# weihaoysgs/ssvio

Measured on AMD Instinct MI355X. Metric: stereo frames/s (ORB extract + row-band match + triangulate + one local BA per frame) on 1241x376, higher is better.
Workload: dtype u8 (front-end) + f64 (BA)

## Files before the change

ssvio_amd/csrc/ba.hip:

```cpp
#include <algorithm>
#include <atomic>
#include <chrono>
#include <cmath>
#include <limits>
#include <map>
#include <condition_variable>
#include <functional>
#include <mutex>
#include <numeric>
#include <thread>
#include <unordered_map>
#include <vector>

#include <cstring>
#include <rocprim/device/device_radix_sort.hpp>
#include <rocprim/device/device_run_length_encode.hpp>
#include <rocprim/device/device_scan.hpp>

#include "ctx.hpp"
#include "se3.hpp"
#include "../../include/ssx_test_hooks.h"

int ssx_comm_allreduce_f64(void* user, double* buf_dev, size_t count, void* stream);

// ... 45 lines not shown
using gcdouble_p = const double*;
#endif


struct BaDev {
  int P, L, E, nP, nLm, nCh, nBlk, world, rank;
  int big;
  int store_w;
  int lin_stride;
  int dense_slabs;
  GPtr<unsigned int> touch;
  GPtr<const int> pose_free;
  GPtr<const uint8_t> lm_fixed;
  GPtr<const int> lm_id;
  GPtr<const int> lm_ptr;
  GPtr<const int> ch_lm;
  GPtr<const int> e_pose;
  GPtr<const int> e_lmc;
  GPtr<const uint8_t> e_cam;
  GPtr<const uint8_t> e_dup;
  GPtr<const double> e_uv;
  GPtr<const int8_t> blk_pa;
  GPtr<const int8_t> blk_pb;
  GPtr<const int4> ch_desc;
  GPtr<const int4> e_rec;
  GPtr<const int4> l_rec;
  GPtr<const uint16_t> pptr;
  GPtr<uint8_t> pair_a;
  GPtr<uint8_t> pair_b;
  GPtr<int> pair_ptr;
  GPtr<int4> bseg;
  GPtr<int> bseg_ptr;
  int bseg_cap;
  int dev_prep;
  int E_raw;
  GPtr<const int> r_edge_pose;
  GPtr<const int> r_edge_point;
  GPtr<const double> r_edge_uv;
  GPtr<const uint8_t> r_edge_cam;
  GPtr<const uint8_t> r_slot8;
  int no_err;
  int raw_fmt;
  GPtr<const int> lm_compact;
  GPtr<const int> pose_rank;
  GPtr<int> perm;
  GPtr<int> lm_chunk;
// ... 134 lines not shown

template <int K0, int N>
__device__ __forceinline__ void pose_terms(const double* Ji, double w, double r0, double r1, double* V)
{
  int k = 0;
#pragma unroll
  for (int r = 0; r < 6; ++r)
#pragma unroll
    for (int cc = r; cc < 6; ++cc) {
      if (k >= K0 && k < K0 + N) V[k - K0] = Ji[r] * w * Ji[cc] + Ji[6 + r] * w * Ji[6 + cc];
      ++k;
    }
#pragma unroll
  for (int a = 0; a < 6; ++a) {
    if (k >= K0 && k < K0 + N) V[k - K0] = Ji[a] * r0 + Ji[6 + a] * r1;
    ++k;
  }
}

__device__ __forceinline__ double run_sum(const double* row, int s0, int s1)
{
  double acc = 0.0;
  int s = s0;
  for (; s < s1; s += 8) {
    double v[8];
#pragma unroll
    for (int i = 0; i < 8; ++i) v[i] = row[s + i];
#pragma unroll
    for (int i = 0; i < 8; ++i) acc += (s + i < s1) ? v[i] : 0.0;
  }
  return acc;
}

__device__ __forceinline__ bool chunk_touches(const BaDev& d, int c, int bit)
{
  return d.dense_slabs || ((d.touch[(size_t)c * TOUCH_WORDS + (bit >> 5)] >> (bit & 31)) & 1u);
}

template <int JAC>
__device__ __forceinline__ void k_linearize_body(const BaDev& d, const int bx, int cur, char* smem, const ChunkLists& cl, double* Wout, double* lmout,
                                                 int* erw_out, double* slab)
{
  double (*sL)[CH_E + 1] = reinterpret_cast<double (*)[CH_E + 1]>(smem);
  double* sV = reinterpret_cast<double*>(smem) + 9 * (CH_E + 1);
  double* sRed = reinterpret_cast<double*>(smem);
  const uint16_t* sPptr = reinterpret_cast<const uint16_t*>(smem + BA_OFF_PPTR);

// ... 603 lines not shown
  if (!both) {
#pragma unroll
    for (int k = 0; k < 18; ++k) W[k] = 0.0;
    return;
  }
  const double* pose = d.pose[cur];
  const double* point = d.point[cur];
  double T[7], X[3];
#pragma unroll
  for (int k = 0; k < 7; ++k) T[k] = pose[p * 7 + k];
#pragma unroll
  for (int k = 0; k < 3; ++k) X[k] = point[lid * 3 + k];
  const double* ext = d.ext + 7 * (er4.w & 1);
  double er[2], p1[3], pc[3], Ji[12], Jj[6], rho0, w;
  ssx::edge_error(T, X, ext, d.K, d.e_uv[e], d.e_uv[d.E + e], er, p1, pc);
  ssx::edge_jac_analytic(T, ext, d.K, p1, pc, Ji, Jj);
  ssx::huber(er[0] * er[0] + er[1] * er[1], d.huber_delta, rho0, w);
#pragma unroll
  for (int a = 0; a < 6; ++a)
#pragma unroll
    for (int b = 0; b < 3; ++b) W[a * 3 + b] = Ji[a] * w * Jj[b] + Ji[6 + a] * w * Jj[3 + b];
}

__device__ __forceinline__ void k_schur_body(const BaDev& d, const int bx, int cur, double lambda, char* smem, const ChunkLists& cl, const double* Win,
                                             const double* lmin, const int* erw_in, double* slab)
{
  double* sY = reinterpret_cast<double*>(smem);
  double* sG = sY + 18 * PW;
  double* sGb = sG + 6 * PL;
  int* sLm = reinterpret_cast<int*>(sGb + 3 * PL);
  const uint16_t* sPptr = reinterpret_cast<const uint16_t*>(smem + BA_OFF_PPTR);
  const uint16_t* sPab = reinterpret_cast<const uint16_t*>(smem + BA_OFF_PAB);

  const int t = tid_opaque();
  (void)bx;
  const int4 cd = cl.cd;
  const int e0 = cd.x, ne = cd.y, lm0 = cd.z, nl = cd.w;
  const int nP = d.nP;

  bool leader = false;
  double Wm[18];
  double z[6] = {0.0, 0.0, 0.0, 0.0, 0.0, 0.0};
  int zpos = 0;
  const int it0 = cl.it0, n_items = cl.n_items;
  int4 item_rec = cl.item_rec;
  if (t < ne) {
    const int e = e0 + t;
    const int erw = erw_in ? *erw_in : d.e_rec[e].w;
    sLm[t] = (erw >> 8) & 0xFF;
    zpos = (erw >> 16) & 0xFF;
    leader = !(erw & (6 | 32));
    if (leader) {
      if (Win) {
#pragma unroll
        for (int k = 0; k < 18; ++k) Wm[k] = Win[k];
      } else if (d.store_w) {
#pragma unroll
        for (int k = 0; k < 18; ++k) Wm[k] = d.W[(size_t)k * d.E + e];
      } else {
        edge_W(d, cur, e, Wm);
      }
      for (int j = t + 1; (erw & 8) && j < ne && d.e_dup[e0 + j]; ++j) {
        double Wd[18];
        if (d.store_w) {
#pragma unroll
          for (int k = 0; k < 18; ++k) Wd[k] = d.W[(size_t)k * d.E + e0 + j];
        } else {
          edge_W(d, cur, e0 + j, Wd);
        }
#pragma unroll
        for (int k = 0; k < 18; ++k) Wm[k] += Wd[k];
      }
    }
  }
  if (t < nl) {
    const int lc = lm0 + t;
    double D[6];
#pragma unroll
    for (int k = 0; k < 6; ++k) D[k] = lmin ? lmin[k] : d.Hll[(size_t)k * d.nLm + lc];
    D[0] += lambda; D[3] += lambda; D[5] += lambda;
    const double i00 = 1.0 / sqrt(D[0]);
    const double l10 = D[1] * i00, l20 = D[2] * i00;
    const double i11 = 1.0 / sqrt(D[3] - l10 * l10);
    const double l21 = (D[4] - l20 * l10) * i11;
    const double i22 = 1.0 / sqrt(D[5] - l20 * l20 - l21 * l21);
    sG[t] = i00; sG[PL + t] = l10; sG[2 * PL + t] = l20; sG[3 * PL + t] = i11; sG[4 * PL + t] = l21; sG[5 * PL + t] = i22;
    const double b0 = lmin ? lmin[6] : d.bl[lc], b1 = lmin ? lmin[7] : d.bl[(size_t)d.nLm + lc], b2 = lmin ? lmin[8] : d.bl[(size_t)2 * d.nLm + lc];
    const double g0 = b0 * i00, g1 = (b1 - l10 * g0) * i11, g2 = (b2 - l20 * g0 - l21 * g1) * i22;
    sGb[t] = g0; sGb[PL + t] = g1; sGb[2 * PL + t] = g2;
  }
  __syncthreads();
  if (t < ne) {
    if (leader) {
      const int l = sLm[t];
      const double i00 = sG[l], l10 = sG[PL + l], l20 = sG[2 * PL + l], i11 = sG[3 * PL + l], l21 = sG[4 * PL + l], i22 = sG[5 * PL + l];
      const double g0 = sGb[l], g1 = sGb[PL + l], g2 = sGb[2 * PL + l];
#pragma unroll
      for (int a = 0; a < 6; ++a) {
        const double y0 = Wm[a * 3] * i00;
        const double y1 = (Wm[a * 3 + 1] - y0 * l10) * i11;
        const double y2 = (Wm[a * 3 + 2] - y0 * l20 - y1 * l21) * i22;
        sY[(a * 3) * PW + t] = y0; sY[(a * 3 + 1) * PW + t] = y1; sY[(a * 3 + 2) * PW + t] = y2;
        z[a] = y0 * g0 + y1 * g1 + y2 * g2;
      }
    } else {
#pragma unroll
      for (int k = 0; k < 18; ++k) sY[k * PW + t] = 0.0;
    }
  }
  __syncthreads();
// ... 6 lines not shown
    const int q0 = ir.y, q1 = ir.z, part = ir.w & 15, parts = ir.w >> 4;
    double acc[3][3];
#pragma unroll
    for (int i = 0; i < 3; ++i)
#pragma unroll
      for (int j = 0; j < 3; ++j) acc[i][j] = 0.0;
    const double* bdp = sY + (qr * 9) * PW;
    const double* wp = sY + (qc * 9) * PW;
#pragma unroll 2
    for (int q = q0; q < q1; ++q) {
      const int ab = sPab[q];
      const int ea = ab & 0xFF, eb = ab >> 8;
      double bd[3][3], w[3][3];
#pragma unroll
      for (int i = 0; i < 3; ++i)
#pragma unroll
        for (int m = 0; m < 3; ++m) { bd[i][m] = bdp[(i * 3 + m) * PW + ea]; w[i][m] = wp[(i * 3 + m) * PW + eb]; }
#pragma unroll
      for (int i = 0; i < 3; ++i)
#pragma unroll
        for (int j = 0; j < 3; ++j) acc[i][j] = fma(bd[i][2], w[j][2], fma(bd[i][1], w[j][1], fma(bd[i][0], w[j][0], acc[i][j])));
    }
    if (__any(parts > 1)) {
#pragma unroll
      for (int i = 0; i < 3; ++i)
#pragma unroll
        for (int j = 0; j < 3; ++j) {
          const double v1 = dpp_f64<0x104>(acc[i][j]), v2 = dpp_f64<0x108>(acc[i][j]), v3 = dpp_f64<0x10C>(acc[i][j]);
          if (part == 0) {
            if (parts > 1) acc[i][j] += v1;
            if (parts > 2) acc[i][j] += v2;
            if (parts > 3) acc[i][j] += v3;
          }
        }
    }
    if (blk >= 0 && part == 0) {
#pragma unroll
      for (int i = 0; i < 3; ++i)
#pragma unroll
        for (int j = 0; j < 3; ++j) slab[blk * 36 + (3 * qr + i) * 6 + 3 * qc + j] = acc[i][j];
    }
  }
  __syncthreads();
  if (t < ne) {
#pragma unroll
    for (int a = 0; a < 6; ++a) sY[a * PW + zpos] = z[a];
  }
  __syncthreads();
  for (int base = 0; base < nP * 6 * 4; base += CH) {
    const int item = base + t;
    const bool on = item < nP * 6 * 4;
    const int idx = on ? item >> 2 : 0, part = item & 3;
    const int p = idx / 6, a = idx - p * 6;
    double acc = 0.0;
    const int s0 = on ? sPptr[p] : 0, s1 = on ? sPptr[p + 1] : 0;
    for (int s = s0 + part; s < s1; s += 4) acc += sY[a * PW + s];
    acc += dpp_f64<DPP_QUAD_XOR1>(acc);
    acc += dpp_f64<DPP_QUAD_XOR2>(acc);
    if (on && part == 0 && (d.dense_slabs || s1 > s0)) slab[nS + idx] = acc;
  }
}

__device__ __forceinline__ void k_schur_entry(const BaDev& d, int bx)
{
  extern __shared__ __attribute__((aligned(16))) char schur_smem[];
  ChunkLists cl;
  chunk_lists_load(d, bx, schur_smem, true, cl);
  if (d.scal[SC_STOP] != 0.0) return;
  const int cur = (int)d.scal[SC_CUR];
  const double lambda = d.scal[SC_LAMBDA];
  k_schur_body(d, bx, cur, lambda, schur_smem, cl, nullptr, nullptr, nullptr, d.schur_slab + (size_t)bx * (d.nBlk * 36 + d.nP * 6));
}
__global__ __launch_bounds__(CH) void k_schur(BaDev d) { k_schur_entry(d, blockIdx.x); }
__global__ __launch_bounds__(CH) void k_schur_b(const BaDev* __restrict__ dv)
{
  const BaDev& d = dv[blockIdx.y];
  if ((int)blockIdx.x >= d.nCh) return;
  k_schur_entry(d, blockIdx.x);
}

template <int JAC>
__device__ __forceinline__ void k_lin_schur_entry(const BaDev& d, int bx)
{
  extern __shared__ __attribute__((aligned(16))) char fused_smem[];
  const double stop = d.scal[SC_STOP], curd = d.scal[SC_CUR], lambda = d.scal[SC_LAMBDA], needlin = d.scal[SC_NEEDLIN];
  ChunkLists cl;
  chunk_lists_load(d, bx, fused_smem, true, cl);
  if (stop != 0.0) return;
  const int cur = (int)curd;
  double* lslab = d.lin_slab + (size_t)bx * d.lin_stride;
  double* sslab = d.schur_slab + (size_t)bx * (d.nBlk * 36 + d.nP * 6);
  if (needlin != 0.0) {
    double W[18], lm[9];
    int erw = 0;
#pragma unroll
    for (int k = 0; k < 18; ++k) W[k] = 0.0;
#pragma unroll
    for (int k = 0; k < 9; ++k) lm[k] = 0.0;
    k_linearize_body<JAC>(d, bx, cur, fused_smem, cl, W, lm, &erw, lslab);
    __syncthreads();
    k_schur_body(d, bx, cur, lambda, fused_smem, cl, W, lm, &erw, sslab);
  } else {
    k_schur_body(d, bx, cur, lambda, fused_smem, cl, nullptr, nullptr, nullptr, sslab);
  }
}
template <int JAC>
__global__ __launch_bounds__(CH, SSX_LS_WGS) void k_lin_schur(BaDev d) { k_lin_schur_entry<JAC>(d, blockIdx.x); }
template <int JAC>
__global__ __launch_bounds__(CH, SSX_LS_WGS) void k_lin_schur_b(const BaDev* __restrict__ dv)
{
  const BaDev& d = dv[blockIdx.y];
  if ((int)blockIdx.x >= d.nCh) return;
  k_lin_schur_entry<JAC>(d, blockIdx.x);
}

template <bool OWN_LIN>
__device__ __forceinline__ void k_reduce_schur_body(const BaDev& d, const int bx)
{
  __shared__ double sAcc[3][64];
  __shared__ double sAccL[3][64];
  __shared__ unsigned int sMask[MASK_TILE * TOUCH_WORDS];
  const int nS = d.nBlk * 36;
  const int stride = nS + d.nP * 6;
  const int n = 6 * d.nP;
  const int t = threadIdx.x;
  const int ent = bx * 64 + (t & 63), grp = t >> 6;
  const int bit = ent < nS ? ent / 36 : d.nBlk + (ent - nS) / 6;
  int lin_ent = -1, lin_pose = 0;
  if (OWN_LIN && ent < stride) {
    if (ent < nS) {
      const int blk = ent / 36, rc = ent - blk * 36;
      const int r = rc / 6, cc = rc - r * 6;
      const int pa = d.blk_pa[blk];
      if (pa == d.blk_pb[blk]) {
        const int rr = r < cc ? r : cc, c2 = r < cc ? cc : r;
        lin_pose = pa;
        lin_ent = pa * 27 + rr * 6 - (rr * (rr - 1)) / 2 + (c2 - rr);
      }
    } else {
      const int j = ent - nS;
      lin_pose = j / 6;
      lin_ent = lin_pose * 27 + UPPER6 + (j - 6 * lin_pose);
    }
  }
  double acc = 0.0, accl = 0.0;
  for (int cb = 0; cb < d.nCh; cb += MASK_TILE) {
    if (cb) __syncthreads();
    stage_masks(d, cb, sMask);
    __syncthreads();
    if (ent < stride) acc = slab_sum_masked(d, d.schur_slab + ent, stride, grp, bit, cb, sMask, acc);
    if (OWN_LIN && lin_ent >= 0) accl = slab_sum_masked(d, d.lin_slab + lin_ent, d.nP * 27 + 2, grp, d.nBlk + lin_pose, cb, sMask, accl);
  }
  if (grp > 0) { sAcc[grp - 1][t & 63] = acc; if (OWN_LIN) sAccL[grp - 1][t & 63] = accl; }
  __syncthreads();
  if (grp != 0 || ent >= stride) return;
  acc = ((acc + sAcc[0][t]) + sAcc[1][t]) + sAcc[2][t];
  if (OWN_LIN) accl = ((accl + sAccL[0][t]) + sAccL[1][t]) + sAccL[2][t];
  double* S = d.trial_comm;
  double* bs = d.trial_comm + (size_t)n * n;
  if (ent < nS) {
    const int blk = ent / 36, rc = ent - blk * 36;
    const int r = rc / 6, cc = rc - r * 6;
    const int pa = d.blk_pa[blk], pb = d.blk_pb[blk];
    double h = 0.0;
    if (pa == pb) {
      const int rr = r < cc ? r : cc, c2 = r < cc ? cc : r;
      const int k = rr * 6 - (rr * (rr - 1)) / 2 + (c2 - rr);
      h = OWN_LIN ? accl : d.Hpp[pa * UPPER6 + k];
    }
    const double v = h - acc;
    S[(size_t)(6 * pa + r) * n + 6 * pb + cc] = v;
    if (pa != pb) S[(size_t)(6 * pb + cc) * n + 6 * pa + r] = v;
  } else {
    const int j = ent - nS;
    bs[j] = (OWN_LIN ? accl : d.bp[j]) - acc;
  }
}

__global__ __launch_bounds__(CH) void k_reduce_schur(BaDev d) { k_reduce_schur_body<false>(d, blockIdx.x); }
__global__ __launch_bounds__(CH) void k_reduce_both(BaDev d, int n_rl)
{
  if ((int)blockIdx.x < n_rl) k_reduce_lin_body(d, blockIdx.x);
  else k_reduce_schur_body<true>(d, blockIdx.x - n_rl);
}
__global__ __launch_bounds__(CH) void k_reduce_both_b(const BaDev* __restrict__ dv, int max_rl)
{
  const BaDev& d = dv[blockIdx.y];
  if ((int)blockIdx.x < max_rl) {
    if ((int)blockIdx.x >= ((d.nP * 27 + 63) / 64 > 0 ? (d.nP * 27 + 63) / 64 : 1)) return;
    k_reduce_lin_body(d, blockIdx.x);
  } else {
    const int bx = (int)blockIdx.x - max_rl;
    if (bx >= ((d.nBlk * 36 + d.nP * 6 + 63) / 64)) return;
    k_reduce_schur_body<true>(d, bx);
  }
}
__global__ __launch_bounds__(CH) void k_reduce_schur_b(const BaDev* __restrict__ dv)
{
  const BaDev& d = dv[blockIdx.y];
// ... 285 lines not shown
inline int dense_slabs_mode()
{
  int m = g_dense_slabs.load(std::memory_order_relaxed);
  if (m < 0) {
    m = getenv("SSX_BA_DENSE_SLABS") ? 1 : 0;
    g_dense_slabs.store(m, std::memory_order_relaxed);
  }
  return m;
}
struct HostPrep {
  int P, L, E, nP, nLm, nCh, nBlk;
  int E_raw = 0;
  int raw_fmt = 0;
  bool big = false;
  bool dev_lists = false;
  bool dev_prep = false;
  int band_w = -1;
  std::vector<int> pose_free, lm_id, lm_ptr, ch_lm;
  std::vector<uint8_t> lm_fixed, slot8;
  std::vector<int> lm_compact;
  std::vector<int> pose_rank;
  std::vector<int> ch_desc;
  std::vector<int8_t> blk_pa, blk_pb;
  std::vector<int> e_pose, e_lmc, perm, pair_ptr;
  std::vector<uint8_t> e_cam, e_dup, pair_a, pair_b;
  std::vector<uint16_t> pptr;
  std::vector<double> e_uv;
  std::vector<int> e_rec, l_rec;
  std::vector<int> lm_chunk;
  std::vector<int> bseg, bseg_ptr;
  std::vector<unsigned int> touch;
  std::vector<int> pe_ptr, pe_edge, sblk_pa, sblk_pb, spair_ptr;
  std::vector<int> thr_cnt, thr_pe, cnt_tmp, start_tmp, first_pf_tmp, visit_tmp, visit2_tmp;
  std::vector<uint32_t> tmp_pairs;
  std::vector<std::pair<int, int>> tmp_order;
};
}

static int host_threads_cap()
{
  static const int cap = [] { const char* e = getenv("SSX_HOST_THREADS"); const int v = e ? atoi(e) : 0; return v > 0 ? std::min(v, 128) : 16; }();
  return cap;
}

class ParPool {
 public:
// ... 825 lines not shown
  return best;
}

uint64_t ssx_ba_debug_prepare_digest(const ssx_ba_problem* prob, int32_t threads)
{
  if (!prob) return 0;
  ssx_ctx dummy;
  static BaWorkspace* wsl = new BaWorkspace();
  dummy.ba = wsl;
  static thread_local HostPrep h;
  g_prep_threads_override = threads;
  const ssx_status st = prepare(&dummy, prob, h);
  g_prep_threads_override = 0;
  dummy.ba = nullptr;
  if (st != SSX_OK) return 0;
  uint64_t d = 1469598103934665603ull;
  auto eat = [&](const void* p, size_t n) { const uint8_t* b = (const uint8_t*)p; for (size_t i = 0; i < n; ++i) { d ^= b[i]; d *= 1099511628211ull; } };
  auto eat_v = [&](const auto& v, size_t n) { n = std::min(n, v.size()); eat(&n, sizeof(n)); eat(v.data(), sizeof(v[0]) * n); };
  const size_t all = ~size_t(0), ref = h.dev_prep ? 0 : all;
  const int sc[13] = {h.P, h.L, h.E, h.E_raw, h.nP, h.nLm, h.nCh, h.nBlk, h.raw_fmt, h.big, h.dev_lists, h.dev_prep, h.band_w};
  eat(sc, sizeof(sc));
  eat_v(h.lm_ptr, all); eat_v(h.lm_id, all); eat_v(h.slot8, h.dev_prep ? h.E_raw : 0); eat_v(h.pe_ptr, all); eat_v(h.ch_lm, all);
  eat_v(h.pose_free, all); eat_v(h.lm_fixed, all); eat_v(h.lm_compact, all); eat_v(h.pose_rank, all); eat_v(h.ch_desc, 4 * (size_t)h.nCh);
  eat_v(h.blk_pa, all); eat_v(h.blk_pb, all);
  eat_v(h.e_pose, ref); eat_v(h.e_lmc, ref); eat_v(h.e_cam, ref); eat_v(h.e_dup, ref); eat_v(h.e_uv, ref); eat_v(h.perm, all);
  eat_v(h.e_rec, std::min(ref, 4 * (size_t)h.E)); eat_v(h.l_rec, std::min(ref, 4 * (size_t)h.nLm)); eat_v(h.lm_chunk, std::min(ref, (size_t)h.nLm));
  eat_v(h.pptr, all); eat_v(h.pair_a, all); eat_v(h.pair_b, all); eat_v(h.pair_ptr, all); eat_v(h.bseg, all); eat_v(h.bseg_ptr, all);
  eat_v(h.touch, (ref && !h.big) ? all : 0);
  eat_v(h.pe_edge, all); eat_v(h.sblk_pa, all); eat_v(h.sblk_pb, all); eat_v(h.spair_ptr, all);
  BandPlan bands[2];
  if (h.big) { plan_band(h.nP, 3, bands[1]); plan_bcr(h.nP, 3, bands[1].bcr); }
  const WinExt win;
  for (int v = 0; v < (h.dev_prep && !h.big ? 3 : 2); ++v)
   for (int keep_init = 0; keep_init < 2; ++keep_init)
    for (int b = 0; b < (h.big ? 2 : 1); ++b) {
      const ArenaPlan p = plan_arena(prob, h, bands[b], v == 1 ? 2 : 1, keep_init != 0, v == 2 ? &win : nullptr, h.big && h.dev_prep);
      for (const Span* s = p.spans_begin(); s != p.spans_end(); ++s) eat(&s->off, sizeof(size_t));
      eat(&p.in_bytes, sizeof(size_t)); eat(&p.total, sizeof(size_t));
    }
  return d;
}

int32_t ssx_ba_debug_upload_format(const ssx_ba_problem* prob)
{
  if (!prob) return -1;
  ssx_ctx dummy;
  static thread_local HostPrep h;
// ... 10 lines not shown
```

ssvio_amd/csrc/ba_marshal.inc:

```

void make_chunks(HostPrep& h)
{
  h.ch_lm.clear();
  h.ch_lm.push_back(0);
  int acc_e = 0, acc_l = 0;
  for (int lc = 0; lc < h.nLm; ++lc) {
    const int k = h.lm_ptr[lc + 1] - h.lm_ptr[lc];
    if (acc_e + k > CH_E || acc_l + 1 > CH_L) {
      h.ch_lm.push_back(lc);
      acc_e = 0; acc_l = 0;
    }
    acc_e += k; acc_l += 1;
  }
  if (h.nLm > 0) h.ch_lm.push_back(h.nLm);
  h.nCh = (int)h.ch_lm.size() - 1;
  if (h.nCh < 0) h.nCh = 0;
}

struct WinExt {
  const int* r_edge_pose = nullptr; const int* r_edge_point = nullptr; const double* r_edge_uv = nullptr; const uint8_t* r_edge_cam = nullptr;
  double* pose[2] = {nullptr, nullptr}; double* point[2] = {nullptr, nullptr};
  int cur = 0;
  const int* pose_order = nullptr; int n_pose_order = 0;
  const int* lm_order = nullptr; int n_lm_order = 0;
// ... 148 lines not shown
  make_chunks(h);
  h.ch_desc.resize(4 * (size_t)std::max(h.nCh, 1));
  for (int c = 0; c < h.nCh; ++c) {
    const int lm0 = h.ch_lm[c], lm1 = h.ch_lm[c + 1], e0 = h.lm_ptr[lm0], e1 = h.lm_ptr[lm1];
    int* cd = &h.ch_desc[4 * (size_t)c];
    cd[0] = e0; cd[1] = e1 - e0; cd[2] = lm0; cd[3] = lm1 - lm0;
  }
}

void prep_drop_reference(HostPrep& h)
{
  h.blk_pa.clear(); h.blk_pb.clear();
  h.band_w = -1;
  h.perm.clear(); h.pptr.clear(); h.pair_ptr.clear(); h.pair_a.clear(); h.pair_b.clear(); h.bseg.clear(); h.bseg_ptr.clear();
  h.pe_edge.clear(); h.sblk_pa.clear(); h.sblk_pb.clear(); h.spair_ptr.assign(1, 0);
}

void prep_small_blocks(HostPrep& h)
{
  h.blk_pa.clear(); h.blk_pb.clear();
  for (int a = 0; a < h.nP; ++a)
    for (int b = a; b < h.nP; ++b) { h.blk_pa.push_back((int8_t)a); h.blk_pb.push_back((int8_t)b); }
  h.nBlk = (int)h.blk_pa.size();
}

void ref_pose_major(HostPrep& h);
ssx_status prep_big_tail(ssx_ctx* ctx, HostPrep& h)
{
  if (h.nP > 2048) { ctx->set_error("ssx_ba: %d free poses exceed the supported 2048", h.nP); return SSX_ERR_UNSUPPORTED; }
  if (h.dev_prep) for (int p = 0; p < h.nP; ++p) h.pe_ptr[p + 1] += h.pe_ptr[p];
  else ref_pose_major(h);
  h.blk_pa.clear(); h.blk_pb.clear();
  h.sblk_pa.clear(); h.sblk_pb.clear(); h.spair_ptr.assign(1, 0);
  h.nBlk = 0;
  h.band_w = -1;
  h.bseg.clear(); h.bseg_ptr.clear();
  h.dev_lists = false;
  return SSX_OK;
}


void ref_sort_columns(const ssx_ba_problem* pr, HostPrep& h)
{
  const int L = h.L, E = h.E;
  h.perm.assign(E, 0);
  {
// ... 206 lines not shown
    bp.seg_m[k] = base + (k < rem ? 1 : 0);
    p += bp.seg_m[k] + w;
  }
}


struct Span { size_t off = 0, n = 0; };

struct ArenaPlan {
  int P, L, E, E_raw, nP, nLm, nCh, nBlk, nBlkS, n, n_pad, lin_stride, bseg_cap, raw_fmt;
  int bw, bK, bnPr, bwr, LS0, LS1, bcrN, bcrm;
  bool big;
  bool on_dev;
  bool dev_prep;
  bool dev_lists;
  bool host_recs;
  bool ext;
  bool raw_in;
  bool cam_in;
  bool have_rank;
  bool keep_init;
  bool band, bcr;
  size_t in_bytes, total;
  Span pose_free, lm_fixed, lm_id, lm_ptr, ch_lm, e_pose, e_lmc, e_cam, e_dup, e_uv, ch_desc, e_rec, l_rec, blk_pa, blk_pb, pptr, lm_compact, pose_rank,
       r_pose, r_point, r_uv, r_cam, slot8, pair_a, pair_b, pair_ptr, bseg, bseg_ptr, touch, pe_ptr, pe_edge, sblk_pa, sblk_pb, spair_ptr, seg_p0, seg_m,
       bcr_p0, bcr_elim, pose0, point0,
       pose1, point1, pose_init, point_init, perm, c2, W, err_lin, err_trial, Hll, bl, lin_slab, Hpp, bp, iter, schur, trial_comm, BDa, Wma, Cv, S, Sb,
       U, Ls0, Sr, Ls1, bcr_mem, xr, x, Ld, invd, Ninv, scale_part, xp, trial, scal_comm, scal, lmstat, ticket;
  const Span* spans_begin() const { return &pose_free; }
  const Span* spans_end() const { return &ticket + 1; }
};
static_assert(offsetof(ArenaPlan, ticket) - offsetof(ArenaPlan, pose_free) == 78 * sizeof(Span), "ArenaPlan: the spans are one run of 79 Span members");

ArenaPlan plan_arena(const ssx_ba_problem* pr, const HostPrep& h, const BandPlan& bp, int world, bool keep_init, const WinExt* ext, bool on_dev)
{
  ArenaPlan p{};
  const int P = p.P = h.P, L = p.L = h.L, E = p.E = h.E, nP = p.nP = h.nP, nLm = p.nLm = h.nLm, nCh = p.nCh = h.nCh, nBlk = p.nBlk = h.nBlk;
  const int E_raw = p.E_raw = h.E_raw, n = p.n = 6 * nP;
  const bool big = p.big = h.big, rz = p.on_dev = on_dev;
  const bool dev_prep = p.dev_prep = h.dev_prep && !big, dev_lists = p.dev_lists = h.dev_lists && !big;
  const bool host_recs = p.host_recs = !dev_prep && !rz, host_lists = !dev_lists;
  const bool big_up = big && !rz;
  const bool lm_up = (big || dev_prep) && !rz;
  p.ext = ext != nullptr;
  const bool raw_in = p.raw_in = dev_prep && !ext;
  p.cam_in = raw_in && pr->edge_cam != nullptr;
  p.have_rank = dev_prep && !h.pose_rank.empty();
  p.keep_init = keep_init && !ext;
  const bool band = p.band = big && bp.w > 0, bcr = p.bcr = band && bp.bcr.on;
  p.bseg_cap = dev_lists ? 2 * nBlk * BSEG_PARTS + 16 : 0;
  p.lin_stride = big ? 2 : nP * 27 + 2;
  const int n_pad = p.n_pad = big ? ((n + NB - 1) / NB) * NB : 0;
  const size_t nBlkS = h.sblk_pa.size();
  p.nBlkS = (int)nBlkS;
  const int raw_fmt = p.raw_fmt = raw_in ? h.raw_fmt : 0;
  const size_t I = sizeof(int), D = sizeof(double);
  Layout lay;
  auto blob = [&](bool on, size_t nbytes, size_t pad = 0, bool filled = true) { return Span{lay.take(on ? nbytes + pad : 0), on && filled ? nbytes : 0}; };
  auto scratch = [&](size_t nbytes) { return Span{lay.take(nbytes), 0}; };
  p.pose_free = blob(!rz, I * P);
  p.lm_fixed = blob(lm_up, nLm); p.lm_id = blob(lm_up, I * nLm); p.lm_ptr = blob(lm_up, I * (nLm + 1));
  p.ch_lm = blob(big_up, I * (nCh + 1));
  p.e_pose = blob(big_up, I * E); p.e_lmc = blob(big_up, I * E); p.e_cam = blob(big_up, E);
  if (host_recs) { p.e_dup = blob(true, E); p.e_uv = blob(true, D * 2 * E); }
  p.ch_desc = blob(!rz, I * 4 * (size_t)nCh, I * 4);
  if (host_recs) { p.e_rec = blob(true, I * 4 * (size_t)E, I * 4); p.l_rec = blob(true, I * 4 * (size_t)nLm, I * 4); }
  p.blk_pa = blob(true, nBlk, 1); p.blk_pb = blob(true, nBlk, 1);
  if (host_recs) p.pptr = blob(true, sizeof(uint16_t) * h.pptr.size(), sizeof(uint16_t));
  p.lm_compact = blob(dev_prep, I * (size_t)L, I);
  p.pose_rank = blob(p.have_rank, I * (size_t)P);
  { const size_t wp = (raw_fmt & 1) ? 1 : I, wl = (raw_fmt & 2) ? sizeof(uint16_t) : I, wuv = 2 * ((raw_fmt & 4) ? sizeof(float) : D);
    p.r_pose = blob(raw_in, wp * E, wp); p.r_point = blob(raw_in, wl * E, wl); p.r_uv = blob(raw_in, wuv * E, wuv); }
  p.r_cam = blob(p.cam_in, E, 1);
  p.slot8 = blob(dev_prep, E_raw, 1);
  const size_t touch_bytes = big ? 0 : sizeof(unsigned int) * TOUCH_WORDS * (size_t)(nCh + 1);
  if (host_lists) {
    p.pair_a = blob(true, h.pair_a.size(), 1); p.pair_b = blob(true, h.pair_a.size(), 1);
    p.pair_ptr = blob(true, I * h.pair_ptr.size(), I); p.bseg = blob(true, I * h.bseg.size(), I * 4); p.bseg_ptr = blob(true, I * h.bseg_ptr.size(), I);
    if (!big) p.touch = blob(true, touch_bytes);
  }
  p.pe_ptr = blob(!rz, I * h.pe_ptr.size(), I, big); p.pe_edge = blob(!rz, I * h.pe_edge.size(), I, big);
  p.sblk_pa = blob(true, I * nBlkS, I, big); p.sblk_pb = blob(true, I * nBlkS, I, big); p.spair_ptr = blob(true, I * h.spair_ptr.size(), I, big);
  p.seg_p0 = blob(true, I * bp.seg_p0.size(), I, band); p.seg_m = blob(true, I * bp.seg_m.size(), I, band);
  p.bcr_p0 = blob(bcr, I * bp.bcr.p0.size(), I); p.bcr_elim = blob(bcr, I * bp.bcr.elim.size(), I * 4);
  p.pose0 = blob(!ext, D * 7 * P); p.point0 = blob(!ext, D * 3 * L, D * 3);
  p.in_bytes = lay.off;
  if (!ext) { p.pose1 = scratch(D * 7 * P); p.point1 = scratch(D * 3 * (L + 1)); }
  if (p.keep_init) { p.pose_init = scratch(D * 7 * P); p.point_init = scratch(D * 3 * (L + 1)); }
  if (dev_prep) {
    p.e_dup = scratch((size_t)E + 1); p.e_uv = scratch(D * 2 * (size_t)(E + 1));
// ... 26 lines not shown
  p.Sb = scratch(D * (sb_count + 1 + (band ? iter_count + 1 : 0)));
  if (band) p.iter = Span{p.Sb.off + D * sb_count, 0};
  p.U = scratch(band ? D * (size_t)bK * NU * NU : 256);
  p.Ls0 = scratch((band && bK > 1) ? D * (size_t)nP * p.LS0 : 256);
  p.Sr = scratch(D * (sr_count + 1));
  p.Ls1 = scratch(band ? D * (size_t)(bK > 1 ? bnPr : nP) * p.LS1 : 256);
  p.bcr_mem = scratch(bcr ? D * (bcr_mem_doubles(p.bcrN, p.bcrm) + 8) : 256);
  p.xr = scratch(D * (6 * (size_t)bnPr + 8)); p.x = scratch(D * (n_pad + 8)); p.Ld = scratch(D * NB * NB); p.invd = scratch(D * (n_pad + 8));
  p.Ninv = scratch(D * 4 * 256); p.scale_part = scratch(D * 64); p.xp = scratch(D * (n + 1)); p.trial = scratch(D * 3 * (nCh + 1));
  p.scal_comm = scratch(D * 4); p.scal = scratch(D * SC_N); p.lmstat = scratch(D * 3 * SSX_BA_MAX_STATS); p.ticket = scratch(sizeof(unsigned int) * 4);
  p.total = lay.off;
  return p;
}

void fill_blob(const ArenaPlan& p, const ssx_ba_problem* pr, const HostPrep& h, const BandPlan& bp, char* hs)
{
  auto put = [&](const Span& s, const void* src) { if (s.n) memcpy(hs + s.off, src, s.n); };
  put(p.pose_free, h.pose_free.data());
  put(p.lm_fixed, h.lm_fixed.data()); put(p.lm_id, h.lm_id.data()); put(p.lm_ptr, h.lm_ptr.data());
  put(p.ch_lm, h.ch_lm.data());
  put(p.e_pose, h.e_pose.data()); put(p.e_lmc, h.e_lmc.data()); put(p.e_cam, h.e_cam.data());
  put(p.e_dup, h.e_dup.data()); put(p.e_uv, h.e_uv.data());
  put(p.ch_desc, h.ch_desc.data()); put(p.e_rec, h.e_rec.data()); put(p.l_rec, h.l_rec.data());
  put(p.blk_pa, h.blk_pa.data()); put(p.blk_pb, h.blk_pb.data());
  put(p.pptr, h.pptr.data());
  put(p.lm_compact, h.lm_compact.data()); put(p.pose_rank, h.pose_rank.data());
  if (p.r_pose.n && (p.raw_fmt & 1)) { uint8_t* o = (uint8_t*)(hs + p.r_pose.off); for (int e = 0; e < p.E; ++e) o[e] = (uint8_t)pr->edge_pose[e]; }
  else put(p.r_pose, pr->edge_pose);
  if (p.r_point.n && (p.raw_fmt & 2)) { uint16_t* o = (uint16_t*)(hs + p.r_point.off); for (int e = 0; e < p.E; ++e) o[e] = (uint16_t)pr->edge_point[e]; }
  else put(p.r_point, pr->edge_point);
  if (p.r_uv.n && (p.raw_fmt & 4)) { float* o = (float*)(hs + p.r_uv.off); for (size_t i = 0; i < 2 * (size_t)p.E; ++i) o[i] = (float)pr->edge_uv[i]; }
  else put(p.r_uv, pr->edge_uv);
  put(p.r_cam, pr->edge_cam);
  put(p.slot8, h.slot8.data());
  put(p.pair_a, h.pair_a.data()); put(p.pair_b, h.pair_b.data()); put(p.pair_ptr, h.pair_ptr.data());
  put(p.bseg, h.bseg.data()); put(p.bseg_ptr, h.bseg_ptr.data()); put(p.touch, h.touch.data());
  put(p.pe_ptr, h.pe_ptr.data()); put(p.pe_edge, h.pe_edge.data());
  put(p.sblk_pa, h.sblk_pa.data()); put(p.sblk_pb, h.sblk_pb.data()); put(p.spair_ptr, h.spair_ptr.data());
  put(p.seg_p0, bp.seg_p0.data()); put(p.seg_m, bp.seg_m.data());
  put(p.bcr_p0, bp.bcr.p0.data()); put(p.bcr_elim, bp.bcr.elim.data());
  put(p.pose0, pr->poses); put(p.point0, pr->points);
}

void wire_arena(const ArenaPlan& p, char* base_in, char* base_rest, const ssx_ba_problem* pr, double huber_delta, double chi2_th, int world, int rank,
                const WinExt* ext, const BaDev* recs, const int* pe_ptr_dev, const int* pe_edge_dev, BaDev& d, BigDev& bd, BandDev& bnd)
{
  auto at = [&](const Span& s) -> char* { return s.off < p.in_bytes ? base_in + s.off : base_rest + (s.off - p.in_bytes); };
  auto at_if = [&](bool on, const Span& s) -> char* { return on ? at(s) : nullptr; };
  d.P = p.P; d.L = p.L; d.E = p.E; d.nP = p.nP; d.nLm = p.nLm; d.nCh = p.nCh; d.nBlk = p.nBlk; d.world = world; d.rank = rank;
  d.big = p.big ? 1 : 0; d.lin_stride = p.lin_stride;
  d.dense_slabs = dense_slabs_mode();
  d.touch = (unsigned int*)at(p.touch);
  d.store_w = 1;
  d.pose_free = (const int*)at(p.pose_free); d.ch_lm = (const int*)at(p.ch_lm);
  d.lm_fixed = (const uint8_t*)at(p.lm_fixed); d.lm_id = (const int*)at(p.lm_id); d.lm_ptr = (const int*)at(p.lm_ptr);
  d.e_pose = (const int*)at(p.e_pose); d.e_lmc = (const int*)at(p.e_lmc); d.e_cam = (const uint8_t*)at(p.e_cam);
  d.e_dup = (const uint8_t*)at(p.e_dup); d.e_uv = (const double*)at(p.e_uv);
  d.ch_desc = (const int4*)at(p.ch_desc); d.e_rec = (const int4*)at(p.e_rec); d.l_rec = (const int4*)at(p.l_rec);
  d.blk_pa = (const int8_t*)at(p.blk_pa); d.blk_pb = (const int8_t*)at(p.blk_pb); d.pptr = (const uint16_t*)at(p.pptr);
  d.pair_a = (uint8_t*)at(p.pair_a); d.pair_b = (uint8_t*)at(p.pair_b); d.pair_ptr = (int*)at(p.pair_ptr);
  d.bseg = (int4*)at(p.bseg); d.bseg_ptr = (int*)at(p.bseg_ptr);
  d.bseg_cap = p.bseg_cap; d.dev_prep = p.dev_prep ? 1 : 0; d.E_raw = p.E_raw; d.raw_fmt = p.raw_fmt;
  d.no_err = 0;
  if (p.ext) {
    d.r_edge_pose = ext->r_edge_pose; d.r_edge_point = ext->r_edge_point; d.r_edge_uv = ext->r_edge_uv; d.r_edge_cam = ext->r_edge_cam;
    d.pose[0] = ext->pose[0]; d.pose[1] = ext->pose[1]; d.point[0] = ext->point[0]; d.point[1] = ext->point[1];
  } else {
    d.r_edge_pose = (const int*)at_if(p.dev_prep, p.r_pose); d.r_edge_point = (const int*)at_if(p.dev_prep, p.r_point);
    d.r_edge_uv = (const double*)at_if(p.dev_prep, p.r_uv); d.r_edge_cam = (const uint8_t*)at_if(p.cam_in, p.r_cam);
    d.pose[0] = (double*)at(p.pose0); d.pose[1] = (double*)at(p.pose1); d.point[0] = (double*)at(p.point0); d.point[1] = (double*)at(p.point1);
  }
  d.r_slot8 = (const uint8_t*)at_if(p.dev_prep, p.slot8); d.lm_compact = (const int*)at_if(p.dev_prep, p.lm_compact);
  d.perm = (int*)at_if(p.dev_prep, p.perm); d.c2_out = (double*)at_if(p.dev_prep, p.c2);
  d.pose_rank = (const int*)at_if(p.have_rank, p.pose_rank);
  d.K = Cam{pr->K[0], pr->K[1], pr->K[2], pr->K[3]};
  for (int i = 0; i < 14; ++i) d.ext[i] = pr->cam_ext[i];
  d.huber_delta = huber_delta; d.chi2_th = chi2_th;
  d.pose_init = (const double*)at_if(p.keep_init, p.pose_init); d.point_init = (const double*)at_if(p.keep_init, p.point_init);
  d.W = (double*)at(p.W); d.err_lin = (double*)at(p.err_lin); d.err_trial = (double*)at(p.err_trial);
  d.Hll = (double*)at(p.Hll); d.bl = (double*)at(p.bl); d.lin_slab = (double*)at(p.lin_slab);
  d.Hpp = (double*)at(p.Hpp); d.bp = (double*)at(p.bp); d.iter_comm = (double*)at(p.iter);
  d.schur_slab = (double*)at(p.schur); d.trial_comm = (double*)at(p.trial_comm); d.xp = (double*)at(p.xp); d.trial_slab = (double*)at(p.trial);
// ... 278 lines not shown
```

Before: 18670.

## Precompute Schur reduction index table and trim branches in Schur body

Adds a host-built per-entry table (output indices, linear-slab index, touch bits) uploaded with the arena, so the Schur reduction kernel reads one int4 instead of doing integer divisions and block-pair lookups. The Schur body also gets an explicit have_in flag instead of null-pointer checks, moves the duplicate-edge merge behind a wave-uniform vote, and only issues the DPP partial-merge shifts that some lane needs. run_sum gains a fast path without per-element bounds masks. The table adds host prep and upload bytes and is only built for non-big problems.

```diff
diff --git a/ssvio_amd/csrc/ba.hip b/ssvio_amd/csrc/ba.hip
--- a/ssvio_amd/csrc/ba.hip
+++ b/ssvio_amd/csrc/ba.hip
@@ -91,6 +91,7 @@
   GPtr<const double> e_uv;
   GPtr<const int8_t> blk_pa;
   GPtr<const int8_t> blk_pb;
+  GPtr<const int4> red_tab;
   GPtr<const int4> ch_desc;
   GPtr<const int4> e_rec;
   GPtr<const int4> l_rec;
@@ -271,7 +272,14 @@
 {
   double acc = 0.0;
   int s = s0;
-  for (; s < s1; s += 8) {
+  for (; s + 8 <= s1; s += 8) {
+    double v[8];
+#pragma unroll
+    for (int i = 0; i < 8; ++i) v[i] = row[s + i];
+#pragma unroll
+    for (int i = 0; i < 8; ++i) acc += v[i];
+  }
+  if (s < s1) {
     double v[8];
 #pragma unroll
     for (int i = 0; i < 8; ++i) v[i] = row[s + i];
@@ -921,8 +929,24 @@
     for (int b = 0; b < 3; ++b) W[a * 3 + b] = Ji[a] * w * Jj[b] + Ji[6 + a] * w * Jj[3 + b];
 }
 
-__device__ __forceinline__ void k_schur_body(const BaDev& d, const int bx, int cur, double lambda, char* smem, const ChunkLists& cl, const double* Win,
-                                             const double* lmin, const int* erw_in, double* slab)
+template <int CTRL>
+__device__ __forceinline__ void part_merge_shift(double (&acc)[3][3], bool on)
+{
+  double v[3][3];
+#pragma unroll
+  for (int i = 0; i < 3; ++i)
+#pragma unroll
+    for (int j = 0; j < 3; ++j) v[i][j] = dpp_f64<CTRL>(acc[i][j]);
+  if (on) {
+#pragma unroll
+    for (int i = 0; i < 3; ++i)
+#pragma unroll
+      for (int j = 0; j < 3; ++j) acc[i][j] += v[i][j];
+  }
+}
+
+__device__ __forceinline__ void k_schur_body(const BaDev& d, const int bx, int cur, double lambda, char* smem, const ChunkLists& cl, const bool have_in,
+                                             const double* Win, const double* lmin, const int* erw_in, double* slab)
 {
   double* sY = reinterpret_cast<double*>(smem);
   double* sG = sY + 18 * PW;
@@ -938,6 +962,7 @@
   const int nP = d.nP;
 
   bool leader = false;
+  int erw_dup = 0;
   double Wm[18];
   double z[6] = {0.0, 0.0, 0.0, 0.0, 0.0, 0.0};
   int zpos = 0;
@@ -945,12 +970,15 @@
   int4 item_rec = cl.item_rec;
   if (t < ne) {
     const int e = e0 + t;
-    const int erw = erw_in ? *erw_in : d.e_rec[e].w;
+    int erw;
+    if (have_in) erw = *erw_in;
+    else erw = d.e_rec[e].w;
     sLm[t] = (erw >> 8) & 0xFF;
     zpos = (erw >> 16) & 0xFF;
     leader = !(erw & (6 | 32));
+    erw_dup = erw;
     if (leader) {
-      if (Win) {
+      if (have_in) {
 #pragma unroll
         for (int k = 0; k < 18; ++k) Wm[k] = Win[k];
       } else if (d.store_w) {
@@ -959,7 +987,11 @@
       } else {
         edge_W(d, cur, e, Wm);
       }
-      for (int j = t + 1; (erw & 8) && j < ne && d.e_dup[e0 + j]; ++j) {
+    }
+  }
+  if (__builtin_expect(__any(leader && (erw_dup & 8)), 0)) {
+    if (leader) {
+      for (int j = t + 1; (erw_dup & 8) && j < ne && d.e_dup[e0 + j]; ++j) {
         double Wd[18];
         if (d.store_w) {
 #pragma unroll
@@ -976,7 +1008,7 @@
     const int lc = lm0 + t;
     double D[6];
 #pragma unroll
-    for (int k = 0; k < 6; ++k) D[k] = lmin ? lmin[k] : d.Hll[(size_t)k * d.nLm + lc];
+    for (int k = 0; k < 6; ++k) D[k] = have_in ? lmin[k] : d.Hll[(size_t)k * d.nLm + lc];
     D[0] += lambda; D[3] += lambda; D[5] += lambda;
     const double i00 = 1.0 / sqrt(D[0]);
     const double l10 = D[1] * i00, l20 = D[2] * i00;
@@ -984,7 +1016,7 @@
     const double l21 = (D[4] - l20 * l10) * i11;
     const double i22 = 1.0 / sqrt(D[5] - l20 * l20 - l21 * l21);
     sG[t] = i00; sG[PL + t] = l10; sG[2 * PL + t] = l20; sG[3 * PL + t] = i11; sG[4 * PL + t] = l21; sG[5 * PL + t] = i22;
-    const double b0 = lmin ? lmin[6] : d.bl[lc], b1 = lmin ? lmin[7] : d.bl[(size_t)d.nLm + lc], b2 = lmin ? lmin[8] : d.bl[(size_t)2 * d.nLm + lc];
+    const double b0 = have_in ? lmin[6] : d.bl[lc], b1 = have_in ? lmin[7] : d.bl[(size_t)d.nLm + lc], b2 = have_in ? lmin[8] : d.bl[(size_t)2 * d.nLm + lc];
     const double g0 = b0 * i00, g1 = (b1 - l10 * g0) * i11, g2 = (b2 - l20 * g0 - l21 * g1) * i22;
     sGb[t] = g0; sGb[PL + t] = g1; sGb[2 * PL + t] = g2;
   }
@@ -1037,17 +1069,10 @@
         for (int j = 0; j < 3; ++j) acc[i][j] = fma(bd[i][2], w[j][2], fma(bd[i][1], w[j][1], fma(bd[i][0], w[j][0], acc[i][j])));
     }
     if (__any(parts > 1)) {
-#pragma unroll
-      for (int i = 0; i < 3; ++i)
-#pragma unroll
-        for (int j = 0; j < 3; ++j) {
-          const double v1 = dpp_f64<0x104>(acc[i][j]), v2 = dpp_f64<0x108>(acc[i][j]), v3 = dpp_f64<0x10C>(acc[i][j]);
-          if (part == 0) {
-            if (parts > 1) acc[i][j] += v1;
-            if (parts > 2) acc[i][j] += v2;
-            if (parts > 3) acc[i][j] += v3;
-          }
-        }
+      const bool first = part == 0;
+      part_merge_shift<0x104>(acc, first && parts > 1);
+      if (__any(parts > 2)) part_merge_shift<0x108>(acc, first && parts > 2);
+      if (__any(parts > 3)) part_merge_shift<0x10C>(acc, first && parts > 3);
     }
     if (blk >= 0 && part == 0) {
 #pragma unroll
@@ -1084,7 +1109,7 @@
   if (d.scal[SC_STOP] != 0.0) return;
   const int cur = (int)d.scal[SC_CUR];
   const double lambda = d.scal[SC_LAMBDA];
-  k_schur_body(d, bx, cur, lambda, schur_smem, cl, nullptr, nullptr, nullptr, d.schur_slab + (size_t)bx * (d.nBlk * 36 + d.nP * 6));
+  k_schur_body(d, bx, cur, lambda, schur_smem, cl, false, nullptr, nullptr, nullptr, d.schur_slab + (size_t)bx * (d.nBlk * 36 + d.nP * 6));
 }
 __global__ __launch_bounds__(CH) void k_schur(BaDev d) { k_schur_entry(d, blockIdx.x); }
 __global__ __launch_bounds__(CH) void k_schur_b(const BaDev* __restrict__ dv)
@@ -1114,9 +1139,9 @@
     for (int k = 0; k < 9; ++k) lm[k] = 0.0;
     k_linearize_body<JAC>(d, bx, cur, fused_smem, cl, W, lm, &erw, lslab);
     __syncthreads();
-    k_schur_body(d, bx, cur, lambda, fused_smem, cl, W, lm, &erw, sslab);
+    k_schur_body(d, bx, cur, lambda, fused_smem, cl, true, W, lm, &erw, sslab);
   } else {
-    k_schur_body(d, bx, cur, lambda, fused_smem, cl, nullptr, nullptr, nullptr, sslab);
+    k_schur_body(d, bx, cur, lambda, fused_smem, cl, false, nullptr, nullptr, nullptr, sslab);
   }
 }
 template <int JAC>
@@ -1135,61 +1160,33 @@
   __shared__ double sAcc[3][64];
   __shared__ double sAccL[3][64];
   __shared__ unsigned int sMask[MASK_TILE * TOUCH_WORDS];
-  const int nS = d.nBlk * 36;
-  const int stride = nS + d.nP * 6;
-  const int n = 6 * d.nP;
+  const int stride = d.nBlk * 36 + d.nP * 6;
   const int t = threadIdx.x;
   const int ent = bx * 64 + (t & 63), grp = t >> 6;
-  const int bit = ent < nS ? ent / 36 : d.nBlk + (ent - nS) / 6;
-  int lin_ent = -1, lin_pose = 0;
-  if (OWN_LIN && ent < stride) {
-    if (ent < nS) {
-      const int blk = ent / 36, rc = ent - blk * 36;
-      const int r = rc / 6, cc = rc - r * 6;
-      const int pa = d.blk_pa[blk];
-      if (pa == d.blk_pb[blk]) {
-        const int rr = r < cc ? r : cc, c2 = r < cc ? cc : r;
-        lin_pose = pa;
-        lin_ent = pa * 27 + rr * 6 - (rr * (rr - 1)) / 2 + (c2 - rr);
-      }
-    } else {
-      const int j = ent - nS;
-      lin_pose = j / 6;
-      lin_ent = lin_pose * 27 + UPPER6 + (j - 6 * lin_pose);
-    }
-  }
+  int4 rt = make_int4(0, -1, -1, 0);
+  if (ent < stride) rt = d.red_tab[ent];
+  const int bit = rt.w & 0xFFFF, lin_ent = OWN_LIN ? rt.z : -1, lin_bit = rt.w >> 16;
   double acc = 0.0, accl = 0.0;
   for (int cb = 0; cb < d.nCh; cb += MASK_TILE) {
     if (cb) __syncthreads();
     stage_masks(d, cb, sMask);
     __syncthreads();
     if (ent < stride) acc = slab_sum_masked(d, d.schur_slab + ent, stride, grp, bit, cb, sMask, acc);
-    if (OWN_LIN && lin_ent >= 0) accl = slab_sum_masked(d, d.lin_slab + lin_ent, d.nP * 27 + 2, grp, d.nBlk + lin_pose, cb, sMask, accl);
+    if (OWN_LIN && lin_ent >= 0) accl = slab_sum_masked(d, d.lin_slab + lin_ent, d.nP * 27 + 2, grp, lin_bit, cb, sMask, accl);
   }
   if (grp > 0) { sAcc[grp - 1][t & 63] = acc; if (OWN_LIN) sAccL[grp - 1][t & 63] = accl; }
   __syncthreads();
   if (grp != 0 || ent >= stride) return;
   acc = ((acc + sAcc[0][t]) + sAcc[1][t]) + sAcc[2][t];
   if (OWN_LIN) accl = ((accl + sAccL[0][t]) + sAccL[1][t]) + sAccL[2][t];
-  double* S = d.trial_comm;
-  double* bs = d.trial_comm + (size_t)n * n;
-  if (ent < nS) {
-    const int blk = ent / 36, rc = ent - blk * 36;
-    const int r = rc / 6, cc = rc - r * 6;
-    const int pa = d.blk_pa[blk], pb = d.blk_pb[blk];
-    double h = 0.0;
-    if (pa == pb) {
-      const int rr = r < cc ? r : cc, c2 = r < cc ? cc : r;
-      const int k = rr * 6 - (rr * (rr - 1)) / 2 + (c2 - rr);
-      h = OWN_LIN ? accl : d.Hpp[pa * UPPER6 + k];
-    }
-    const double v = h - acc;
-    S[(size_t)(6 * pa + r) * n + 6 * pb + cc] = v;
-    if (pa != pb) S[(size_t)(6 * pb + cc) * n + 6 * pa + r] = v;
-  } else {
-    const int j = ent - nS;
-    bs[j] = (OWN_LIN ? accl : d.bp[j]) - acc;
-  }
+  double h = 0.0;
+  if (rt.z >= 0) {
+    if (OWN_LIN) h = accl;
+    else { const int p = rt.z / 27, k = rt.z - p * 27; h = k < UPPER6 ? d.Hpp[p * UPPER6 + k] : d.bp[p * 6 + (k - UPPER6)]; }
+  }
+  const double v = h - acc;
+  d.trial_comm[rt.x] = v;
+  if (rt.y >= 0) d.trial_comm[rt.y] = v;
 }
 
 __global__ __launch_bounds__(CH) void k_reduce_schur(BaDev d) { k_reduce_schur_body<false>(d, blockIdx.x); }
@@ -1521,6 +1518,8 @@
   std::vector<int> pose_rank;
   std::vector<int> ch_desc;
   std::vector<int8_t> blk_pa, blk_pb;
+  std::vector<int> red_tab;
+  int red_tab_nP = -1;
   std::vector<int> e_pose, e_lmc, perm, pair_ptr;
   std::vector<uint8_t> e_cam, e_dup, pair_a, pair_b;
   std::vector<uint16_t> pptr;
@@ -2392,7 +2391,7 @@
   eat(sc, sizeof(sc));
   eat_v(h.lm_ptr, all); eat_v(h.lm_id, all); eat_v(h.slot8, h.dev_prep ? h.E_raw : 0); eat_v(h.pe_ptr, all); eat_v(h.ch_lm, all);
   eat_v(h.pose_free, all); eat_v(h.lm_fixed, all); eat_v(h.lm_compact, all); eat_v(h.pose_rank, all); eat_v(h.ch_desc, 4 * (size_t)h.nCh);
-  eat_v(h.blk_pa, all); eat_v(h.blk_pb, all);
+  eat_v(h.blk_pa, all); eat_v(h.blk_pb, all); eat_v(h.red_tab, h.big ? 0 : all);
   eat_v(h.e_pose, ref); eat_v(h.e_lmc, ref); eat_v(h.e_cam, ref); eat_v(h.e_dup, ref); eat_v(h.e_uv, ref); eat_v(h.perm, all);
   eat_v(h.e_rec, std::min(ref, 4 * (size_t)h.E)); eat_v(h.l_rec, std::min(ref, 4 * (size_t)h.nLm)); eat_v(h.lm_chunk, std::min(ref, (size_t)h.nLm));
   eat_v(h.pptr, all); eat_v(h.pair_a, all); eat_v(h.pair_b, all); eat_v(h.pair_ptr, all); eat_v(h.bseg, all); eat_v(h.bseg_ptr, all);
diff --git a/ssvio_amd/csrc/ba_marshal.inc b/ssvio_amd/csrc/ba_marshal.inc
--- a/ssvio_amd/csrc/ba_marshal.inc
+++ b/ssvio_amd/csrc/ba_marshal.inc
@@ -194,6 +194,26 @@
   for (int a = 0; a < h.nP; ++a)
     for (int b = a; b < h.nP; ++b) { h.blk_pa.push_back((int8_t)a); h.blk_pb.push_back((int8_t)b); }
   h.nBlk = (int)h.blk_pa.size();
+  if (h.red_tab_nP == h.nP) return;
+  const int nP = h.nP, nS = 36 * h.nBlk, n = 6 * nP;
+  h.red_tab.resize(4 * ((size_t)nS + n));
+  int* rt = h.red_tab.data();
+  for (int blk = 0; blk < h.nBlk; ++blk) {
+    const int pa = h.blk_pa[blk], pb = h.blk_pb[blk];
+    for (int r = 0; r < 6; ++r)
+      for (int cc = 0; cc < 6; ++cc, rt += 4) {
+        const int rr = std::min(r, cc), c2 = std::max(r, cc);
+        rt[0] = (6 * pa + r) * n + 6 * pb + cc;
+        rt[1] = pa != pb ? (6 * pb + cc) * n + 6 * pa + r : -1;
+        rt[2] = pa == pb ? pa * 27 + rr * 6 - (rr * (rr - 1)) / 2 + (c2 - rr) : -1;
+        rt[3] = blk | (pa == pb ? (h.nBlk + pa) << 16 : 0);
+      }
+  }
+  for (int j = 0; j < n; ++j, rt += 4) {
+    const int p = j / 6;
+    rt[0] = n * n + j; rt[1] = -1; rt[2] = p * 27 + UPPER6 + (j - 6 * p); rt[3] = (h.nBlk + p) | (h.nBlk + p) << 16;
+  }
+  h.red_tab_nP = nP;
 }
 
 void ref_pose_major(HostPrep& h);
@@ -446,7 +466,7 @@
   bool keep_init;
   bool band, bcr;
   size_t in_bytes, total;
-  Span pose_free, lm_fixed, lm_id, lm_ptr, ch_lm, e_pose, e_lmc, e_cam, e_dup, e_uv, ch_desc, e_rec, l_rec, blk_pa, blk_pb, pptr, lm_compact, pose_rank,
+  Span pose_free, lm_fixed, lm_id, lm_ptr, ch_lm, e_pose, e_lmc, e_cam, e_dup, e_uv, ch_desc, e_rec, l_rec, blk_pa, blk_pb, red_tab, pptr, lm_compact, pose_rank,
        r_pose, r_point, r_uv, r_cam, slot8, pair_a, pair_b, pair_ptr, bseg, bseg_ptr, touch, pe_ptr, pe_edge, sblk_pa, sblk_pb, spair_ptr, seg_p0, seg_m,
        bcr_p0, bcr_elim, pose0, point0,
        pose1, point1, pose_init, point_init, perm, c2, W, err_lin, err_trial, Hll, bl, lin_slab, Hpp, bp, iter, schur, trial_comm, BDa, Wma, Cv, S, Sb,
@@ -454,7 +474,7 @@
   const Span* spans_begin() const { return &pose_free; }
   const Span* spans_end() const { return &ticket + 1; }
 };
-static_assert(offsetof(ArenaPlan, ticket) - offsetof(ArenaPlan, pose_free) == 78 * sizeof(Span), "ArenaPlan: the spans are one run of 79 Span members");
+static_assert(offsetof(ArenaPlan, ticket) - offsetof(ArenaPlan, pose_free) == 79 * sizeof(Span), "ArenaPlan: the spans are one run of 80 Span members");
 
 ArenaPlan plan_arena(const ssx_ba_problem* pr, const HostPrep& h, const BandPlan& bp, int world, bool keep_init, const WinExt* ext, bool on_dev)
 {
@@ -490,6 +510,7 @@
   p.ch_desc = blob(!rz, I * 4 * (size_t)nCh, I * 4);
   if (host_recs) { p.e_rec = blob(true, I * 4 * (size_t)E, I * 4); p.l_rec = blob(true, I * 4 * (size_t)nLm, I * 4); }
   p.blk_pa = blob(true, nBlk, 1); p.blk_pb = blob(true, nBlk, 1);
+  p.red_tab = blob(!big, I * 4 * (36 * (size_t)nBlk + 6 * (size_t)nP), I * 4);
   if (host_recs) p.pptr = blob(true, sizeof(uint16_t) * h.pptr.size(), sizeof(uint16_t));
   p.lm_compact = blob(dev_prep, I * (size_t)L, I);
   p.pose_rank = blob(p.have_rank, I * (size_t)P);
@@ -562,7 +583,7 @@
   put(p.e_pose, h.e_pose.data()); put(p.e_lmc, h.e_lmc.data()); put(p.e_cam, h.e_cam.data());
   put(p.e_dup, h.e_dup.data()); put(p.e_uv, h.e_uv.data());
   put(p.ch_desc, h.ch_desc.data()); put(p.e_rec, h.e_rec.data()); put(p.l_rec, h.l_rec.data());
-  put(p.blk_pa, h.blk_pa.data()); put(p.blk_pb, h.blk_pb.data());
+  put(p.blk_pa, h.blk_pa.data()); put(p.blk_pb, h.blk_pb.data()); put(p.red_tab, h.red_tab.data());
   put(p.pptr, h.pptr.data());
   put(p.lm_compact, h.lm_compact.data()); put(p.pose_rank, h.pose_rank.data());
   if (p.r_pose.n && (p.raw_fmt & 1)) { uint8_t* o = (uint8_t*)(hs + p.r_pose.off); for (int e = 0; e < p.E; ++e) o[e] = (uint8_t)pr->edge_pose[e]; }
@@ -597,7 +618,7 @@
   d.e_pose = (const int*)at(p.e_pose); d.e_lmc = (const int*)at(p.e_lmc); d.e_cam = (const uint8_t*)at(p.e_cam);
   d.e_dup = (const uint8_t*)at(p.e_dup); d.e_uv = (const double*)at(p.e_uv);
   d.ch_desc = (const int4*)at(p.ch_desc); d.e_rec = (const int4*)at(p.e_rec); d.l_rec = (const int4*)at(p.l_rec);
-  d.blk_pa = (const int8_t*)at(p.blk_pa); d.blk_pb = (const int8_t*)at(p.blk_pb); d.pptr = (const uint16_t*)at(p.pptr);
+  d.blk_pa = (const int8_t*)at(p.blk_pa); d.blk_pb = (const int8_t*)at(p.blk_pb); d.red_tab = (const int4*)at(p.red_tab); d.pptr = (const uint16_t*)at(p.pptr);
   d.pair_a = (uint8_t*)at(p.pair_a); d.pair_b = (uint8_t*)at(p.pair_b); d.pair_ptr = (int*)at(p.pair_ptr);
   d.bseg = (int4*)at(p.bseg); d.bseg_ptr = (int*)at(p.bseg_ptr);
   d.bseg_cap = p.bseg_cap; d.dev_prep = p.dev_prep ? 1 : 0; d.E_raw = p.E_raw; d.raw_fmt = p.raw_fmt;
```

After: 18630. No clear change (-0.2%).
